# intel/pailliercryptolib

Hardware: AMD Instinct MI355X
Metric: 2048-bit modexps/sec (encrypt+decrypt) (higher is better)
Workload: dtype u64

## Files before the change

pailliercryptolib_amd/csrc/capi.cpp:

```cpp
#include "pgpu.h"

#include <hip/hip_runtime_api.h>

#include <algorithm>
#include <atomic>
#include <chrono>
#include <cstdio>
#include <cstdlib>
#include <cstring>
#include <deque>
#include <list>
#include <map>
#include <set>
#include <memory>
#include <mutex>
#include <string>
#include <vector>

#include "ipcl/bignum.h"
#include "kargs.hpp"
#include "launch.hpp"
#include "policy.hpp"
#include "runtime.hpp"

// ... 1490 lines not shown
               hipStream_t s, bool in_mont, const uint32_t* d_pair = nullptr, int in_pair_l2 = 0, int busy_lanes = 0) {
  const int nw = key->n_words;
  if (busy_lanes == 0 && key->hs_ps && hensel_enabled() && secret_policy() != PGPU_EXP_SLIDING &&
      (d_pair ? key->hs_ps->pair_l2 == in_pair_l2 : key->conv_form != nullptr)) {
    if (const size_t head = policy::ps_split_head(key->hs_ps->K, count)) {
      RC_TRY(decrypt_on(d, key, d_c, d_m, head, s, in_mont, d_pair, in_pair_l2, busy_lanes));
      return decrypt_on(d, key, d_c ? d_c + head * (size_t)2 * nw : nullptr, d_m + head * (size_t)nw, count - head, s, in_mont,
                        d_pair ? d_pair + head * (size_t)2 * in_pair_l2 : nullptr, in_pair_l2, busy_lanes);
    }
  }
  rt::StreamWork& w = d.work_for(s);
  std::lock_guard<std::mutex> lk(w.mu);
  RC_TRY(w.vbuf.ensure(2 * count * (size_t)nw * 8, s));
  const bool lat = use_latency_geo(key->geo_lat, key->geo_exp, 2 * count);
  const bool sliding = secret_policy() == PGPU_EXP_SLIDING && key->sched[0].dev.bytes;
  bool have_m = false;
  const pgpu_privkey::HenselSet* hset = pick_hensel(key, count);
  rt::DevMem conv_rows;
  if (!d_pair && !sliding && hset && key->conv_form) {
    const pgpu_privkey::HenselSet* cand = hset;
    const int cl2 = key->conv_form->H * key->conv_form->K;
    if (cand->pair_l2 == cl2 && (seq_form_pays(cand->H, cand->K, count, busy_lanes) || ps_form_pays(key, count, busy_lanes) ||
                                 wave_form_pays(key, count, busy_lanes))) {
      RC_TRY(conv_rows.alloc(d, s, count * (size_t)2 * cl2 * sizeof(uint32_t)));
      RC_TRY(words_to_pair_on(d, key->conv_form.get(), d_c, (size_t)2 * nw, 2 * nw, in_mont, (uint32_t*)conv_rows.p, count, s));
      d_pair = (const uint32_t*)conv_rows.p;
      in_pair_l2 = cl2;
    }
  }
  const bool wavef = d_pair && !sliding && hset && wave_form_pays(key, count, busy_lanes) && key->hs_ps->pair_l2 == in_pair_l2 &&
                     (policy::wave_policy() == 2 || 2 * count * (size_t)(1 + wave_neighbours(d, s)) <= kSimds);
  const bool psf = wavef || (d_pair && !sliding && hset && ps_form_pays(key, count, busy_lanes) &&
                             key->hs_ps->pair_l2 == in_pair_l2);
  if (psf) hset = key->hs_ps.get();
  const pgpu_privkey::HenselSet* bset = (psf && !wavef) ? ps_balanced_set(key, in_pair_l2) : nullptr;
  if (bset) hset = bset;
  if (d_pair && (!hset || hset->pair_l2 != in_pair_l2))
    return fail(PGPU_ERR_UNSUPPORTED, "decrypt: pair-row ciphertexts need the split-form kernel of this key size");
  if (hset) {
    const int L2 = hset->H * hset->K, nch = hset->nchunks, ipw = 64 / (2 * hset->H);
    const size_t side_words = hset->side_words();
    const uint32_t* blob = (const uint32_t*)hset->blob.d[(size_t)d.index];
    pgpu::HenselArgs h{};
    for (int sd = 0; sd < 2; ++sd) {
      const uint32_t* b = blob + sd * side_words;
      h.ctx[sd].nhat = b;
      h.ctx[sd].n = b + L2;
      h.ctx[sd].h = b + 2 * L2;
      h.ctx[sd].kr = b + 3 * L2;
      h.ctx[sd].one = b + 4 * L2;
      h.ctx[sd].conv = b + 6 * L2 + (in_mont ? (size_t)nch * 2 * L2 : 0);
      h.ctx[sd].n0inv = hset->n0inv[sd];
    }
    h.ct = d_c;
    h.ct_stride = (size_t)2 * nw;
    h.ct_words = 2 * nw;
    if (d_pair) {
      h.ct_pair = d_pair;
      h.ct_pair_stride = (size_t)2 * in_pair_l2;
      h.pair_l2 = in_pair_l2;
      h.pchunk_limbs = hset->pchunk_limbs;
      h.pchunks = hset->pchunks;
      for (int sd = 0; sd < 2; ++sd) {
        const uint32_t* pc = blob + sd * side_words + (size_t)L2 * (6 + 4 * (size_t)nch);
        h.ctx[sd].pconv = pc;
        h.ctx[sd].pcb = pc + (size_t)hset->pchunks * 2 * L2;
      }
    }
    h.chunk_words = hset->chunk_words;
    h.nchunks = nch;
    h.exp = (const uint64_t*)key->d_exps.d[(size_t)d.index];
    h.exp_stride = (size_t)key->pq_words;
    h.exp_words = key->pq_words;
    h.exp_bits = key->exp_bits;
    size_t entries;
    if (sliding) {
      for (int i = 0; i < 2; ++i) {
        h.sched[i] = (const uint16_t*)key->sched[i].dev.d[(size_t)d.index];
        h.sched_len[i] = key->sched[i].len;
      }
      h.window = key->sched[0].w;
      entries = (size_t)1 << (h.window - 1);
    } else {
      h.window = g_ct_gather.load() ? std::min(masked_decrypt_window(), pick_window(h.exp_bits)) : policy::pick_decrypt_window(h.exp_bits, 2 * count * (size_t)2 * L2 * sizeof(uint32_t));
      if (wavef) h.window = std::min(h.window, 5);
      entries = (size_t)1 << h.window;
    }
    h.ct_gather = g_ct_gather.load();
    h.out = (uint64_t*)w.vbuf.p;
    h.out_stride = (size_t)key->pq_words;
    h.out_words = key->pq_words;
    h.count = count;
    const size_t waves = 2 * ((count + ipw - 1) / ipw);
    const unsigned blocks = (unsigned)((waves + pgpu::kWavesPerWG - 1) / pgpu::kWavesPerWG);
    TimerScope t(d, s, PGPU_KERNEL_MODEXP);
    const size_t seq_ipw = 64 / (size_t)hset->H;
    const size_t seq_waves = 2 * ((count + seq_ipw - 1) / seq_ipw);
    const bool seq = !psf && d_pair && !sliding && seq_form_pays(hset->H, hset->K, count, busy_lanes);
    t.set_form(psf ? PGPU_FORM_LANE | PGPU_FORM_PS : seq ? PGPU_FORM_SEQ : PGPU_FORM_PAIRED);
    if (wavef) {
      t.set_form(PGPU_FORM_WAVE | PGPU_FORM_PS);
      RC_TRY(w.table.ensure(2 * count * (size_t)(2 * hset->pchunks) * pgpu::hensel_wave_pair_words(hset->K) * sizeof(uint32_t), s));
      h.table = (uint32_t*)w.table.p;
      static const bool wide_ok = [] { const char* e = getenv("PGPU_WAVE_WIDEQ"); return !e || atoi(e) != 0; }();
      const bool wide = wide_ok && hset->lb * hset->K - (key->exp_bits + hset->lb) >= 10;
      if (!pgpu::launch_hensel_wave(hset->K, hset->lb, wide, h, s))
        return fail(PGPU_ERR_UNSUPPORTED, "wavefront-wide decrypt kernel not compiled");
    } else if (psf) {
      const size_t lwaves = 2 * ((count + 63) / 64);
      const unsigned lblocks = (unsigned)((lwaves + pgpu::kWavesPerWG - 1) / pgpu::kWavesPerWG);
      RC_TRY(w.table.ensure((size_t)lblocks * pgpu::kWavesPerWG * pgpu::hensel_ps_table_words(hset->K, entries) * sizeof(uint32_t), s));
      h.table = (uint32_t*)w.table.p;
      const unsigned lds_pad = adaptive_cu_claim(lwaves, busy_lanes);
      if (lds_pad) t.set_form(PGPU_FORM_LANE | PGPU_FORM_PS | PGPU_FORM_CU_CLAIM);
      if (bset ? !pgpu::launch_hensel_psb(hset->K, hset->lb, h, lblocks, s, lds_pad)
               : !pgpu::launch_hensel_ps(hset->K, hset->lb, h, lblocks, s, lds_pad))
        return fail(PGPU_ERR_UNSUPPORTED, "one-lane product-scanning decrypt kernel not compiled");
    } else if (seq) {
      const unsigned sblocks = (unsigned)((seq_waves + pgpu::kWavesPerWG - 1) / pgpu::kWavesPerWG);
      RC_TRY(w.table.ensure((size_t)sblocks * pgpu::kWavesPerWG * seq_ipw * entries * 2 * L2 * sizeof(uint32_t), s));
      h.table = (uint32_t*)w.table.p;
      static const int env_pad = [] {
        const char* e = getenv("PGPU_SEQ_LDS_PAD");
        return e ? atoi(e) : -1;
      }();
      const int pol = policy::seq_policy();
      const unsigned lds_pad = env_pad >= 0 ? (unsigned)env_pad
                               : (seq_waves < kSimds && (pol == 3 || (pol == 4 && busy_lanes >= 1 && busy_lanes <= policy::adapt_claim_busy())) ? 84000u : 0u);
      if (lds_pad) t.set_form(PGPU_FORM_SEQ | PGPU_FORM_CU_CLAIM);
      static const bool w1 = [] { const char* e = getenv("PGPU_SEQ_W1"); return !e || atoi(e) != 0; }();
      if (!pgpu::launch_hensel_seq(hset->H, hset->K, h, sblocks, s, lds_pad, w1 && lds_pad >= 82000u))
        return fail(PGPU_ERR_UNSUPPORTED, "sequential-halves decrypt kernel not compiled");
    } else {
      RC_TRY(w.table.ensure((size_t)blocks * pgpu::kWavesPerWG * ipw * entries * 2 * L2 * sizeof(uint32_t), s));
      h.table = (uint32_t*)w.table.p;
      if (!pgpu::launch_hensel(hset->H, hset->K, waves > kSimds || g_packed_decrypt.load(), h, blocks, s))
        return fail(PGPU_ERR_UNSUPPORTED, "split-form kernel not compiled");
    }
    HIP_TRY(hipGetLastError());
    t.stop();
    have_m = true;
  }
  pgpu::ModexpArgs a{};
  const int vf = in_mont ? VF_BASE_MONT : VF_NONE;
  a.ctx[0] = (lat ? key->p2l : key->p2)->view(d.index, vf);
  a.ctx[1] = (lat ? key->q2l : key->q2)->view(d.index, vf);
  a.nctx = 2;
  a.base = d_c;
  a.base_stride = (size_t)2 * nw;
  a.base_words = 2 * nw;
  a.exp = (const uint64_t*)key->d_exps.d[(size_t)d.index];
  a.exp_stride = (size_t)key->pq_words;
  a.exp_per_ctx = 1;
  a.exp_words = key->pq_words;
  a.exp_bits = key->exp_bits;
  a.final_mul = pgpu::FM_CTX_CONST;
  a.out = (uint64_t*)w.vbuf.p;
  a.out_stride = (size_t)nw;
  a.count = 2 * count;
  SchedRef sr;
  if (sliding) {
    for (int i = 0; i < 2; ++i) {
      sr.p[i] = (const uint16_t*)key->sched[i].dev.d[(size_t)d.index];
      sr.len[i] = key->sched[i].len;
    }
    sr.w = key->sched[0].w;
  }
// ... 378 lines not shown
  *split = 0;
  *lanes = g.G;
  *limbs = g.K;
  return PGPU_OK;
}

int pgpu_decrypt_kernel_form(const pgpu_privkey* key, size_t count, int* split, int* lanes, int* limbs) {
  RC_TRY(pgpu_decrypt_kernel_form_ex(key, count, 0, split, lanes, limbs));
  if (*split == 4 && key->hs_ps) *limbs = key->hs_ps->K;
  return PGPU_OK;
}
int pgpu_decrypt_kernel_form_ex(const pgpu_privkey* key, size_t count, int busy_lanes, int* split, int* lanes, int* limbs) {
  if (!key || !split || !lanes || !limbs) return fail(PGPU_ERR_INVALID_PARAM, "pgpu_decrypt_kernel_form: bad argument");
  RC_TRY(check_gen(key->gen, "key"));
  if (const pgpu_privkey::HenselSet* f = pick_hensel(key, count)) {
    if (pair_rows_enabled() && secret_policy() != PGPU_EXP_SLIDING && wave_form_pays(key, count, busy_lanes) &&
        key->hs_ps->pair_l2 == f->pair_l2) {
      *split = 5;
      *lanes = 64;
      *limbs = key->hs_ps->K;
      return PGPU_OK;
    }
    if (pair_rows_enabled() && secret_policy() != PGPU_EXP_SLIDING && ps_form_pays(key, count, busy_lanes) &&
        key->hs_ps->pair_l2 == f->pair_l2) {
      *split = 4;
      *lanes = 1;
      const pgpu_privkey::HenselSet* bal = ps_balanced_set(key, f->pair_l2);
      *limbs = bal ? bal->K : key->hs_ps->K;
      return PGPU_OK;
    }
    if (pair_rows_enabled() && secret_policy() != PGPU_EXP_SLIDING && seq_form_pays(f->H, f->K, count, busy_lanes)) {
      *split = 2;
      *lanes = f->H;
    } else {
      *split = 1;
      *lanes = 2 * f->H;
    }
    *limbs = f->K;
    return PGPU_OK;
  }
  const bool lat = use_latency_geo(key->geo_lat, key->geo_exp, 2 * count);
  const GeoInfo g = lat ? key->geo_lat : launch_geo(key->geo_exp, 2 * count);
  *split = 0;
  *lanes = g.G;
  *limbs = g.K;
  return PGPU_OK;
}

int pgpu_set_fixed_base_window(int w) {
  if (w < 0 || w > kFbMaxW) return fail(PGPU_ERR_INVALID_PARAM, "fixed-base window must be 0..14");
  g_fb_window.store(w);
  g_fb_window_explicit.store(true);
  return PGPU_OK;
}

int pgpu_set_secret_exponent_policy(int policy) {
  if (policy != PGPU_EXP_FIXED_WINDOW && policy != PGPU_EXP_SLIDING)
    return fail(PGPU_ERR_INVALID_PARAM, "unknown exponent policy");
  g_secret_policy.store(policy);
  return PGPU_OK;
}
int pgpu_get_secret_exponent_policy(void) { return secret_policy(); }
int pgpu_set_table_gather_policy(int masked) {
  g_ct_gather.store(masked ? 1 : 0);
  return PGPU_OK;
}
int pgpu_get_table_gather_policy(void) { return g_ct_gather.load(); }

void pgpu_debug_set_wave_clocks(uint64_t* d_buf) { g_wave_clocks = d_buf; }
void pgpu_debug_set_row_source(int mode) { g_row_source.store(mode < 0 ? -1 : (mode ? 1 : 0)); }
void pgpu_debug_set_hensel(int mode) { g_hensel.store(mode < 0 ? 0 : (mode > 3 ? 3 : mode)); }
void pgpu_debug_set_packed_decrypt(int on) { g_packed_decrypt.store(on != 0); }
void pgpu_debug_set_seq_decrypt(int policy) { pgpu::policy::set_seq_policy(policy); }
int pgpu_debug_set_host_adapt(int on) {
  const int was = g_host_adapt.exchange(on != 0 ? 1 : 0);
  return was;
}
int pgpu_debug_get_seq_decrypt(void) { return pgpu::policy::seq_policy(); }
void pgpu_debug_set_ps_decrypt(int policy) { pgpu::policy::set_ps_policy(policy); }
void pgpu_debug_set_wave_decrypt(int policy) { pgpu::policy::set_wave_policy(policy); }
int pgpu_debug_get_wave_decrypt(void) { return pgpu::policy::wave_policy(); }
int pgpu_debug_get_ps_decrypt(void) { return pgpu::policy::ps_policy(); }
int pgpu_debug_set_ps_balanced(int on) { return g_ps_balanced.exchange(on != 0 ? 1 : 0); }
int pgpu_debug_set_rr_adapt(int min_busy) { return pgpu::policy::set_rr_adapt(min_busy); }

#include "capi_timing.inc"

int pgpu_dev_alloc(size_t bytes, void** out) {
  RC_TRY(rt::check_ready());
  return rt::current().alloc(bytes, nullptr, out);
}
void pgpu_dev_free(void* d_ptr) {
  if (!d_ptr) return;
  if (!rt::initialized()) {
    (void)hipFree(d_ptr);
    return;
  }
  rt::current().free(d_ptr, nullptr);
}
int pgpu_copy_h2d(void* d_dst, const void* h_src, size_t bytes) {
  RC_TRY(rt::check_ready());
  rt::TaskGroup tg;
  tg.run(rt::current(), [=](rt::Lane& lane) -> int {
    HIP_TRY(hipStreamSynchronize(nullptr));
    RC_TRY(lane.h2d(d_dst, h_src, bytes, lane.stream));
    HIP_TRY(hipStreamSynchronize(lane.stream));
    return PGPU_OK;
  });
  return tg.wait();
}
int pgpu_copy_d2h(void* h_dst, const void* d_src, size_t bytes) {
  RC_TRY(rt::check_ready());
  rt::TaskGroup tg;
  tg.run(rt::current(), [=](rt::Lane& lane) -> int {
    hipError_t e = hipStreamSynchronize(nullptr);
    if (e != hipSuccess) return fail(PGPU_ERR_HIP, std::string("kernel failed: ") + hipGetErrorString(e));
    return lane.d2h(h_dst, d_src, bytes, lane.stream);
  });
  return tg.wait();
}

int pgpu_host_alloc(size_t bytes, void** out) { return rt::host_alloc(bytes, out); }
void pgpu_host_free(void* p) { rt::host_free(p); }
int pgpu_host_wait(const void* p) { return rt::host_wait(p); }

int pgpu_modexp_dev(const uint64_t* d_base, size_t base_stride, const uint64_t* d_exp,
                    size_t exp_stride, int exp_words, int exp_bits, const uint64_t* h_mod,
                    int mod_words, uint64_t* d_out, size_t count, void* hip_stream) {
  RC_TRY(rt::check_ready());
  if (count == 0) return PGPU_OK;
  if (!d_base || !d_exp || !d_out) return fail(PGPU_ERR_INVALID_PARAM, "null batch pointer");
  if (exp_words <= 0 || exp_bits < 0 || exp_bits > 64 * exp_words)
    return fail(PGPU_ERR_INVALID_PARAM, "exp_bits/exp_words inconsistent");
  if (base_stride != 0 && base_stride < (size_t)mod_words)
    return fail(PGPU_ERR_INVALID_PARAM, "base stride smaller than the modulus width");
  if (exp_stride != 0 && exp_stride < (size_t)exp_words)
    return fail(PGPU_ERR_INVALID_PARAM, "exponent stride smaller than exp_words");
  rt::Device& d = rt::current();
  rt::DeviceGuard g(d.ordinal);
  return modexp_on(d, d_base, base_stride, d_exp, exp_stride, exp_words, exp_bits, h_mod, mod_words, d_out, count,
                   (hipStream_t)hip_stream, nullptr, false, false, nullptr);
}

int pgpu_modexp(const uint64_t* base, size_t base_stride, const uint64_t* exp, size_t exp_stride,
                int exp_words, int exp_bits, const uint64_t* mod, int mod_words, uint64_t* out,
                size_t count) {
  RC_TRY(rt::check_ready());
  if (count == 0) return PGPU_OK;
  if (!base || !exp || !out || mod_words <= 0 || exp_words <= 0)
    return fail(PGPU_ERR_INVALID_PARAM, "null batch pointer or zero width");
  if (exp_bits < 0 || exp_bits > 64 * exp_words)
    return fail(PGPU_ERR_INVALID_PARAM, "exp_bits/exp_words inconsistent");
  if (base_stride != 0 && base_stride < (size_t)mod_words)
    return fail(PGPU_ERR_INVALID_PARAM, "base stride smaller than the modulus width");
  if (exp_stride != 0 && exp_stride < (size_t)exp_words)
    return fail(PGPU_ERR_INVALID_PARAM, "exponent stride smaller than exp_words");
  std::shared_ptr<ModCtx> ctx;
  RC_TRY(get_modctx(mod, mod_words, true, &ctx));
  std::vector<uint16_t> sched;
  int sched_w = 0;
  if (exp_stride == 0 && count >= 16 && exp_bits > 8 && sliding_enabled()) {
    BigNumber e = BigNumber::fromLimbs64(exp, (size_t)exp_words);
    if (!e.isZero()) {
      sched_w = pick_sliding_window(e.BitSize());
      sched = sliding_schedule(e, sched_w);
    }
// ... 230 lines not shown
```

pailliercryptolib_amd/csrc/hensel_ps.hpp:

```cpp
#ifndef PAILLIERCRYPTOLIB_AMD_CSRC_HENSEL_PS_HPP_
#define PAILLIERCRYPTOLIB_AMD_CSRC_HENSEL_PS_HPP_

#include <utility>

#include "hensel.hpp"

#ifndef PGPU_PS_PIN
#define PGPU_PS_PIN 1
#endif
#ifndef PGPU_PS_SPLIT
#define PGPU_PS_SPLIT 0
#endif

namespace pgpu {

template <int LB>
struct PsLimb {
  static constexpr uint32_t mask = (1u << LB) - 1;
};

template <class F, int... Is>
__device__ __forceinline__ void ps_static_for_impl(F&& f, std::integer_sequence<int, Is...>) {
  (f(std::integral_constant<int, Is>{}), ...);
}
// ... 328 lines not shown
      b[j] = kb[j];
      ma[j] = HCTX(h)[j];
      mb[j] = 0;
    }
  }
  ps_pairmul<K, LB, false>(a, b, ma, mb, np, 0, n0, slot);
  uint32_t d[K];
  const uint32_t below_a = ps_sub<K, LB>(d, a, np);
  const uint32_t jflag = below_a ^ 1u;
  const uint32_t below = ps_sub<K, LB>(d, b, np);
  if (!below) {
#pragma unroll
    for (int j = 0; j < K; ++j) b[j] = d[j];
  }
  (void)ps_sub<K, LB>(d, np, b);
  {
    uint32_t jf[K];
#pragma unroll
    for (int j = 0; j < K; ++j) jf[j] = j == 0 ? jflag : 0u;
    ps_add<K, LB>(d, jf);
  }
  const uint32_t small = ps_sub<K, LB>(b, d, np);
  if (small) {
#pragma unroll
    for (int j = 0; j < K; ++j) b[j] = d[j];
  }
  if (live) {
    uint64_t* out = A.out + (2 * elem + side) * A.out_stride;
    const int ow = A.out_words;
    ps_static_for<W64>([&](auto wc) __attribute__((always_inline)) {
      constexpr int ww = decltype(wc)::value;
      if (ww < ow) out[ww] = ps_word<K, LB, ww>(b);
    });
    for (int ww = W64; ww < ow; ++ww) out[ww] = 0;
  }
#undef HCTX
}

template <int K>
constexpr size_t ps_table_words(size_t entries) { return entries * 2 * ((K + 3) / 4) * kWave * 4; }

template <int K, int LB, int MINW>
__global__ __launch_bounds__(kWGThreads, MINW) void hensel_decrypt_ps_kernel(HenselArgs A) {
  constexpr int K4 = (K + 3) / 4;
  raise_wave_priority();
  __shared__ uint4 park_[kWavesPerWG][K4][kWave];
  const int lane = threadIdx.x % kWave, wv = threadIdx.x / kWave;
  uint4* slot = &park_[wv][0][lane];
  const size_t wave_id = (size_t)blockIdx.x * kWavesPerWG + wv;
  const int side = __builtin_amdgcn_readfirstlane((int)(wave_id & 1));
  const size_t first_elem = (wave_id >> 1) * kWave;
  size_t elem = first_elem + lane;
  if (elem >= A.count) elem = A.count - 1;
#define HCTX(field) (side ? A.ctx[1].field : A.ctx[0].field)
  uint32_t n[K], a[K], b[K], ma[K], mb[K];
#pragma unroll
  for (int j = 0; j < K; ++j) n[j] = ps_uniform(HCTX(nhat)[j]);
  const uint32_t n1p = n[1] + 1;
  const int w = A.window, tsize = 1 << w;
  uint4* tw = reinterpret_cast<uint4*>(A.table + wave_id * ps_table_words<K>((size_t)tsize)) + lane;
  const uint64_t* ep = A.exp + (size_t)side * A.exp_stride;
  const int nwin = (A.exp_bits + w - 1) / w;
  auto digit = [&](int i) -> int {
    int bit = i * w;
    int word = bit >> 6, sh = bit & 63;
    uint64_t v = (word < A.exp_words) ? ep[word] >> sh : 0;
    if (sh + w > 64 && word + 1 < A.exp_words) v |= ep[word + 1] << (64 - sh);
    return (int)(v & (uint64_t)(tsize - 1));
  };
  const bool gather = A.ct_gather != 0;

  ps_entry_from_pair_row<K, LB>(A, side, elem, n, n1p, slot, a, b, ma, mb);
  ps_table_store<K>(tw, 1, a, b);
  {
    uint32_t oa[K], ob[K];
#pragma unroll
    for (int j = 0; j < K; ++j) {
      oa[j] = HCTX(one)[j];
      ob[j] = HCTX(one)[K + j];
    }
    ps_table_store<K>(tw, 0, oa, ob);
  }
#pragma unroll 1
  for (int e = 2; e < tsize; ++e) {
    ps_table_load<K>(ma, mb, tw, 1, tsize, false);
    ps_pairmul<K, LB, true>(a, b, ma, mb, n, n1p, 0, slot);
    ps_table_store<K>(tw, e, a, b);
  }
  int win = nwin - 2;
  if (nwin > 0) {
    ps_table_load<K>(a, b, tw, digit(nwin - 1), tsize, gather);
  } else {
#pragma unroll
    for (int j = 0; j < K; ++j) {
      a[j] = HCTX(one)[j];
      b[j] = HCTX(one)[K + j];
    }
  }
#pragma unroll 1
  for (; nwin > 0 && win >= 0; --win) {
    const int idx = digit(win);
#pragma unroll 1
    for (int i = 0; i < w; ++i) ps_pairsqr<K, LB>(a, b, n, n1p);
    ps_table_load<K>(ma, mb, tw, idx, tsize, gather);
    ps_pairmul<K, LB, true>(a, b, ma, mb, n, n1p, 0, slot);
  }
  ps_exit_words<K, LB>(A, side, elem, first_elem + lane < A.count, slot, a, b, ma, mb);
#undef HCTX
}

}

#endif
```

pailliercryptolib_amd/csrc/hensel_ps_bal.hpp:

```cpp
#ifndef PAILLIERCRYPTOLIB_AMD_CSRC_HENSEL_PS_BAL_HPP_
#define PAILLIERCRYPTOLIB_AMD_CSRC_HENSEL_PS_BAL_HPP_

#include "hensel_ps.hpp"

namespace pgpu {

template <int LB>
__device__ __forceinline__ int32_t psb_sext(uint32_t v) { return __builtin_amdgcn_sbfe((int)v, 0u, (unsigned)LB); }

__device__ __forceinline__ void psb_mac(int64_t& acc, int32_t x, int32_t y) { acc += (int64_t)x * y; }
__device__ __forceinline__ void psb_mac_pinned(int64_t& acc, int32_t x, int32_t y) {
  acc += (int64_t)x * y;
  asm volatile("" ::"v"(acc));
}

template <int K, int LB>
struct PsbFits {
  static constexpr bool value = 2 * (LB - 1) < 62 && LB + 6 < 62 &&
                                3 * (uint64_t)K * ((uint64_t)1 << (2 * (LB - 1))) + ((uint64_t)1 << (LB + 6)) < ((uint64_t)1 << 63);
};

template <int K, int LB, int NP, bool SYM, int QMODE>
__device__ __forceinline__ void psb_montmul(int32_t (&r)[K], const int32_t (&x1)[K], const int32_t (&y1)[K],
                                            const int32_t (&x2)[K], const int32_t (&y2)[K], const int32_t (&n)[K],
                                            uint32_t n0inv, int32_t (&qio)[K]) {
  static_assert(!(SYM && NP != 1), "a symmetric product is a single one");
  static_assert(PsbFits<K, LB>::value, "a column sums up to 3K products below 2^(2(LB-1)): must stay below 2^63");
  int32_t q[K];
  int64_t acc = 0;
  int32_t onev = 1;
  asm("" : "+v"(onev));
  ps_static_for<2 * K>([&](auto colc) __attribute__((always_inline)) {
    constexpr int col = decltype(colc)::value;
    {
      constexpr int ilo = col < K ? 0 : col - K + 1;
      constexpr int ihi = col < K ? col : K;
      if constexpr (ihi > ilo) {
        ps_static_for<ihi - ilo>([&](auto ic) __attribute__((always_inline)) {
          constexpr int i = ilo + decltype(ic)::value;
          if constexpr (PGPU_PS_PIN == 2 || (PGPU_PS_PIN == 1 && SYM)) psb_mac_pinned(acc, q[i], n[col - i]);
          else psb_mac(acc, q[i], n[col - i]);
        });
      }
    }
    if constexpr (SYM) {
      constexpr int ilo = col < K ? 0 : col - K + 1;
      constexpr int ihi = (col + 1) / 2;
      if constexpr (ihi > ilo) {
        int64_t cross = 0;
        ps_static_for<ihi - ilo>([&](auto ic) __attribute__((always_inline)) {
          constexpr int i = ilo + decltype(ic)::value;
          psb_mac(cross, x1[i], x1[col - i]);
        });
        acc = (int64_t)((uint64_t)acc + ((uint64_t)cross << 1));
      }
      if constexpr (col % 2 == 0) psb_mac(acc, x1[col / 2], x1[col / 2]);
    } else {
      constexpr int ilo = col < K ? 0 : col - K + 1;
      constexpr int ihi = col < K ? col + 1 : K;
      ps_static_for<ihi - ilo>([&](auto ic) __attribute__((always_inline)) {
        constexpr int i = ilo + decltype(ic)::value;
        if constexpr (PGPU_PS_PIN == 2) {
          psb_mac_pinned(acc, x1[i], y1[col - i]);
          if constexpr (NP == 2) psb_mac_pinned(acc, x2[i], y2[col - i]);
        } else {
          psb_mac(acc, x1[i], y1[col - i]);
          if constexpr (NP == 2) psb_mac(acc, x2[i], y2[col - i]);
        }
      });
    }
    if constexpr (col < K) {
      if constexpr (QMODE == 2) psb_mac(acc, qio[col], onev);
      q[col] = psb_sext<LB>((uint32_t)acc * n0inv);
      psb_mac(acc, q[col], n[0]);
      acc >>= LB;
      if constexpr (QMODE == 1) qio[col] = q[col];
    } else {
      r[col - K] = psb_sext<LB>((uint32_t)acc);
      if constexpr (col + 1 < 2 * K) acc = (acc + ((int64_t)1 << (LB - 1))) >> LB;
    }
  });
}

template <int K>
__device__ __forceinline__ uint32_t (&psb_bits(int32_t (&v)[K]))[K] { return reinterpret_cast<uint32_t(&)[K]>(v); }
template <int K>
__device__ __forceinline__ const uint32_t (&psb_bits(const int32_t (&v)[K]))[K] { return reinterpret_cast<const uint32_t(&)[K]>(v); }

template <int K, int LB>
__device__ __forceinline__ void psb_pairsqr(int32_t (&a)[K], int32_t (&b)[K], const int32_t (&n)[K], uint32_t n0inv) {
  int32_t qd[K], t[K];
  psb_montmul<K, LB, 1, true, 1>(t, a, a, a, a, n, n0inv, qd);
#pragma unroll
  for (int j = 0; j < K; ++j) b[j] *= 2;
  psb_montmul<K, LB, 1, false, 2>(b, a, b, a, b, n, n0inv, qd);
#pragma unroll
  for (int j = 0; j < K; ++j) a[j] = t[j];
}

template <int K, int LB>
__device__ __forceinline__ void psb_pairmul(int32_t (&a)[K], int32_t (&b)[K], const int32_t (&c)[K], const int32_t (&d)[K],
                                            const int32_t (&n)[K], uint32_t n0inv, uint4* slot) {
  int32_t qd[K];
  {
    int32_t t[K];
    ps_park_store<K>(slot, psb_bits<K>(b));
    __builtin_amdgcn_sched_barrier(0);
    psb_montmul<K, LB, 1, false, 1>(t, a, c, a, c, n, n0inv, qd);
    __builtin_amdgcn_sched_barrier(0);
    ps_park_swap<K>(slot, psb_bits<K>(b), psb_bits<K>(t));
    __builtin_amdgcn_sched_barrier(0);
  }
  psb_montmul<K, LB, 2, false, 2>(b, a, d, b, c, n, n0inv, qd);
  __builtin_amdgcn_sched_barrier(0);
  ps_park_load<K>(psb_bits<K>(a), slot);
}

template <int K, int LB>
__device__ __forceinline__ void psb_mul(int32_t (&r)[K], const int32_t (&x)[K], const int32_t (&y)[K], const int32_t (&n)[K],
                                        uint32_t n0inv) {
  int32_t none[K];
  psb_montmul<K, LB, 1, false, 0>(r, x, y, x, y, n, n0inv, none);
}

template <int K, int LB>
__device__ __forceinline__ void psb_add(int32_t (&a)[K], const int32_t (&k)[K]) {
  int32_t c = 0;
#pragma unroll
  for (int j = 0; j < K; ++j) {
    const int32_t u = a[j] + k[j] + c;
    a[j] = j + 1 < K ? psb_sext<LB>((uint32_t)u) : u;
    c = (u + (1 << (LB - 1))) >> LB;
  }
}

template <int K, int LB, int NI>
__device__ __forceinline__ void psb_relimb(int32_t (&out)[K], const uint32_t (&in)[NI]) {
  static_assert(NI <= K, "the chunk must fit");
  uint32_t c = 0;
#pragma unroll
  for (int j = 0; j < K; ++j) {
    const uint32_t u = (j < NI ? in[j] : 0u) + c;
    out[j] = j + 1 < K ? psb_sext<LB>(u) : (int32_t)u;
    c = (u + (1u << (LB - 1))) >> LB;
  }
}

template <int K, int LB>
__device__ __forceinline__ int32_t psb_canon(uint32_t (&out)[K], const int32_t (&v)[K]) {
  int32_t c = 0;
#pragma unroll
  for (int j = 0; j < K; ++j) {
    const int32_t u = v[j] + c;
    out[j] = (uint32_t)u & PsLimb<LB>::mask;
    c = u >> LB;
  }
  return c;
}

template <int K, int LB>
__device__ __forceinline__ void psb_entry_from_pair_row(const HenselArgs& A, int side, size_t elem, const int32_t (&n)[K],
                                                        uint32_t n0inv, uint4* slot, int32_t (&a)[K], int32_t (&b)[K],
                                                        int32_t (&ma)[K], int32_t (&mb)[K]) {
  static_assert(LB == kLimbBits, "the row limbs are re-balanced, not re-cut");
  constexpr int NI = (K * LB - 2) / LB + 1;
#define HCTX(field) (side ? A.ctx[1].field : A.ctx[0].field)
  const uint32_t* row = A.ct_pair + elem * A.ct_pair_stride;
  int32_t acc_a[K], acc_b[K];
#pragma unroll
  for (int j = 0; j < K; ++j) acc_a[j] = acc_b[j] = 0;
#pragma unroll 1
  for (int i = 0; i < A.pchunks; ++i) {
    const int first = i * A.pchunk_limbs;
    uint32_t za[NI], zb[NI];
    int32_t cb[K], tb[K];
#pragma unroll
    for (int j = 0; j < NI; ++j) {
      const bool in = j < A.pchunk_limbs && first + j < A.pair_l2;
// ... 24 lines not shown
#undef HCTX
}

template <int K, int LB>
__device__ __forceinline__ void psb_exit_words(const HenselArgs& A, int side, size_t elem, bool live, uint4* slot,
                                               const int32_t (&n)[K], uint32_t n0inv, int32_t (&a)[K], int32_t (&b)[K],
                                               int32_t (&ma)[K], int32_t (&mb)[K]) {
  constexpr int W64 = (K * LB + 63) / 64;
#define HCTX(field) (side ? A.ctx[1].field : A.ctx[0].field)
#pragma unroll
  for (int j = 0; j < K; ++j) {
    ma[j] = (int32_t)HCTX(h)[j];
    mb[j] = 0;
  }
  psb_pairmul<K, LB>(a, b, ma, mb, n, n0inv, slot);
  uint32_t u0[K], u1[K];
  const int32_t neg_a = psb_canon<K, LB>(u0, a);
#pragma unroll
  for (int j = 0; j < K; ++j) ma[j] = a[j] - n[j];
  const int32_t below_p = psb_canon<K, LB>(u0, ma);
  const int32_t jflag = (below_p + 1) + neg_a;
#pragma unroll
  for (int j = 0; j < K; ++j) ma[j] = (j == 0 ? jflag : 0) - b[j];
  const int32_t neg_d = psb_canon<K, LB>(u0, ma);
#pragma unroll
  for (int j = 0; j < K; ++j) ma[j] += n[j];
  (void)psb_canon<K, LB>(u1, ma);
#pragma unroll
  for (int j = 0; j < K; ++j) u0[j] = neg_d ? u1[j] : u0[j];
  if (live) {
    uint64_t* out = A.out + (2 * elem + side) * A.out_stride;
    const int ow = A.out_words;
    ps_static_for<W64>([&](auto wc) __attribute__((always_inline)) {
      constexpr int ww = decltype(wc)::value;
      if (ww < ow) out[ww] = ps_word<K, LB, ww>(u0);
    });
    for (int ww = W64; ww < ow; ++ww) out[ww] = 0;
  }
#undef HCTX
}

template <int K, int LB, int MINW>
__global__ __launch_bounds__(kWGThreads, MINW) void hensel_decrypt_psb_kernel(HenselArgs A) {
  constexpr int K4 = (K + 3) / 4;
  raise_wave_priority();
  __shared__ uint4 park_[kWavesPerWG][K4][kWave];
  const int lane = threadIdx.x % kWave, wv = threadIdx.x / kWave;
  uint4* slot = &park_[wv][0][lane];
  const size_t wave_id = (size_t)blockIdx.x * kWavesPerWG + wv;
  const int side = __builtin_amdgcn_readfirstlane((int)(wave_id & 1));
  const size_t first_elem = (wave_id >> 1) * kWave;
  size_t elem = first_elem + lane;
  if (elem >= A.count) elem = A.count - 1;
#define HCTX(field) (side ? A.ctx[1].field : A.ctx[0].field)
  int32_t n[K], a[K], b[K], ma[K], mb[K];
#pragma unroll
  for (int j = 0; j < K; ++j) n[j] = (int32_t)ps_uniform(HCTX(nhat)[j]);
  const uint32_t n0inv = ps_uniform(HCTX(n0inv));
  const int w = A.window, tsize = 1 << w;
  uint4* tw = reinterpret_cast<uint4*>(A.table + wave_id * ps_table_words<K>((size_t)tsize)) + lane;
  const uint64_t* ep = A.exp + (size_t)side * A.exp_stride;
  const int nwin = (A.exp_bits + w - 1) / w;
  auto digit = [&](int i) -> int {
    int bit = i * w;
    int word = bit >> 6, sh = bit & 63;
    uint64_t v = (word < A.exp_words) ? ep[word] >> sh : 0;
    if (sh + w > 64 && word + 1 < A.exp_words) v |= ep[word + 1] << (64 - sh);
    return (int)(v & (uint64_t)(tsize - 1));
  };
  const bool gather = A.ct_gather != 0;

  psb_entry_from_pair_row<K, LB>(A, side, elem, n, n0inv, slot, a, b, ma, mb);
  ps_table_store<K>(tw, 1, psb_bits<K>(a), psb_bits<K>(b));
  {
    uint32_t oa[K], ob[K];
#pragma unroll
    for (int j = 0; j < K; ++j) {
      oa[j] = HCTX(one)[j];
      ob[j] = HCTX(one)[K + j];
    }
    ps_table_store<K>(tw, 0, oa, ob);
  }
#pragma unroll 1
  for (int e = 2; e < tsize; ++e) {
    ps_table_load<K>(psb_bits<K>(ma), psb_bits<K>(mb), tw, 1, tsize, false);
    psb_pairmul<K, LB>(a, b, ma, mb, n, n0inv, slot);
    ps_table_store<K>(tw, e, psb_bits<K>(a), psb_bits<K>(b));
  }
  int win = nwin - 2;
  if (nwin > 0) {
    ps_table_load<K>(psb_bits<K>(a), psb_bits<K>(b), tw, digit(nwin - 1), tsize, gather);
  } else {
#pragma unroll
    for (int j = 0; j < K; ++j) {
      a[j] = (int32_t)HCTX(one)[j];
      b[j] = (int32_t)HCTX(one)[K + j];
    }
  }
#pragma unroll 1
  for (; nwin > 0 && win >= 0; --win) {
    const int idx = digit(win);
#pragma unroll 1
    for (int i = 0; i < w; ++i) psb_pairsqr<K, LB>(a, b, n, n0inv);
    ps_table_load<K>(psb_bits<K>(ma), psb_bits<K>(mb), tw, idx, tsize, gather);
    psb_pairmul<K, LB>(a, b, ma, mb, n, n0inv, slot);
  }
  psb_exit_words<K, LB>(A, side, elem, first_elem + lane < A.count, slot, n, n0inv, a, b, ma, mb);
#undef HCTX
}

}

#endif
```

pailliercryptolib_amd/csrc/policy.cpp:

```cpp
#include "policy.hpp"

#include <algorithm>
#include <atomic>
#include <cstdlib>
#include <utility>

#include "launch.hpp"

namespace pgpu {
namespace policy {

namespace {
int env_int(const char* name, int dflt, int lo, int hi) {
  const char* e = std::getenv(name);
  return e ? std::max(lo, std::min(hi, std::atoi(e))) : dflt;
}
std::atomic<int> g_seq_policy{env_int("PGPU_SEQ_DECRYPT", 4, 0, 4)};
std::atomic<int> g_ps_policy{env_int("PGPU_PS_DECRYPT", 1, 0, 2)};
constexpr int kAdaptEncSeq = 3;
constexpr int kAdaptClaimBusy = 3;
std::atomic<int> g_wave_policy{env_int("PGPU_WAVE_FORMS", 1, 0, 2)};
std::atomic<int> g_rr_adapt{env_int("PGPU_RR_ADAPT", 3, 0, 100)};
}

int seq_policy() { return g_seq_policy.load(); }
void set_seq_policy(int p) { g_seq_policy.store(p < 0 ? 0 : (p > 4 ? 4 : p)); }
int ps_policy() { return g_ps_policy.load(); }
void set_ps_policy(int p) { g_ps_policy.store(p < 0 ? 0 : (p > 2 ? 2 : p)); }
int adapt_claim_busy() { return kAdaptClaimBusy; }
int wave_policy() { return g_wave_policy.load(); }
void set_wave_policy(int p) { g_wave_policy.store(p < 0 ? 0 : (p > 2 ? 2 : p)); }
int rr_adapt() { return g_rr_adapt.load(); }
int set_rr_adapt(int min_busy) { return g_rr_adapt.exchange(min_busy < 0 ? 0 : min_busy); }

int seq_policy_by_size() {
  const int p = g_seq_policy.load();
  return (p == 3 || p == 4) ? 1 : p;
}
bool seq_adaptive(size_t waves, int busy) {
  return g_seq_policy.load() == 4 && busy >= 1 && waves * (size_t)(1 + busy) >= kSimds;
}
unsigned adaptive_cu_claim(size_t waves, int busy_lanes) {
  return (g_seq_policy.load() == 4 && waves < kSimds && busy_lanes >= 1 && busy_lanes <= kAdaptClaimBusy) ? 84000u : 0u;
}

bool fb_encrypt_seq_pays(int H, int K, size_t count, int busy) {
  if (!pgpu::hensel_fb_encrypt_seq_has(H, K)) return false;
  const size_t ipw = 64 / (size_t)H;
  const size_t waves = (count + ipw - 1) / ipw;
  const int pol = seq_policy_by_size();
  if (H == 4 && busy != 2 && busy <= kAdaptEncSeq && seq_adaptive(waves, busy)) return true;
  if (H == 2 && pol != 2) return false;
  return pol == 2 || (pol == 1 && waves >= (H >= 8 ? 2 : 1) * kSimds);
}
bool modexp_seq_form_pays(int H, int K, size_t count) {
  if (!pgpu::hensel_modexp_seq_has(H, K)) return false;
  const size_t ipw = 64 / (size_t)H;
  const size_t waves = (count + ipw - 1) / ipw;
  const int pol = seq_policy_by_size();
  if (H == 2 && pol != 2) return false;
  return pol == 2 || (pol == 1 && waves >= (H >= 8 ? 2 : 1) * kSimds);
}
bool seq_form_pays(int H, int K, size_t count, int busy) {
  if (!pgpu::hensel_seq_has(H, K)) return false;
  const size_t ipw = 64 / (size_t)H;
  const size_t waves = 2 * ((count + ipw - 1) / ipw);
  const int pol = g_seq_policy.load();
  return pol == 2 || (pol == 3 && 2 * waves >= kSimds) || ((pol == 1 || pol == 4) && waves >= kSimds) || seq_adaptive(waves, busy);
}
size_t ps_min_count(int K) {
  return K == 56 ? 24576 + 1 : (K == 38 || K == 19) ? 16384 + 1 : kPsRound;
}
static size_t ps_split_tail(int K) { return K == 56 ? 24576 : 16384; }
bool wave_form_pays(size_t count, int busy) {
  const int pol = g_wave_policy.load();
  if (pol == 2) return true;
  return pol == 1 && g_ps_policy.load() == 1 && busy == 0 && 2 * count <= kSimds;
}
bool modexp_wave_form_pays(size_t count) {
  const int pol = g_wave_policy.load();
  if (pol == 2) return true;
  return pol == 1 && g_ps_policy.load() == 1 && count <= kSimds;
}
bool ps_form_pays(size_t count, int busy, int K) {
  const size_t waves = 2 * ((count + 63) / 64);
  const int pol = g_ps_policy.load();
  return pol == 2 || (pol == 1 && (count >= ps_min_count(K) || seq_adaptive(waves, busy)));
}
size_t ps_split_head(int K, size_t count) {
  if (g_ps_policy.load() != 1 || count <= kPsRound) return 0;
  const size_t tail = count % kPsRound;
  return (tail != 0 && tail <= ps_split_tail(K)) ? count - tail : 0;
}
bool pair_mul_seq_pays(int H, int K, size_t count) {
  if (!pgpu::pair_mul_seq_has(H, K)) return false;
  const size_t ipw = 64 / (size_t)H;
  const size_t waves = (count + ipw - 1) / ipw;
  const int pol = seq_policy_by_size();
  return pol == 2 || (pol == 1 && waves >= (H >= 8 ? 2 : 1) * kSimds);
}

int pick_window(int exp_bits) {
  static const int forced = env_int("PGPU_FIXED_WINDOW", 0, 1, 6);
  if (forced) return forced;
  int best = 1;
  long best_cost = 1L << 60;
  for (int w = 1; w <= 5; ++w) {
    long cost = ((1L << w) - 2) + (exp_bits + w - 1) / w;
    if (cost < best_cost) { best_cost = cost; best = w; }
  }
  return best;
}
constexpr size_t kDecryptTableCap = (size_t)4 << 30;
int pick_decrypt_window(int exp_bits, size_t entry_bytes) {
  const int w5 = pick_window(exp_bits);
  static const int forced = env_int("PGPU_FIXED_WINDOW", 0, 1, 6);
  if (forced || exp_bits < 1280) return w5;
  if (entry_bytes > (kDecryptTableCap >> 6)) return w5;
  const long c5 = ((1L << w5) - 2) + (exp_bits + w5 - 1) / w5, c6 = ((1L << 6) - 2) + (exp_bits + 5) / 6;
  return c6 < c5 ? 6 : w5;
}
int masked_decrypt_window() { return 3; }

static long env_now(const char* name) {
  const char* e = std::getenv(name);
  return e && *e ? std::atol(e) : 0;
}
bool pair_form_for_bits(int n_bits, int* G, int* K) {
  static const int forms[4][2] = {{2, 19}, {4, 18}, {8, 14}, {8, 18}};
  if (n_bits < 1) return false;
  for (const auto& f : forms) {
    if (pgpu::kLimbBits * f[0] * f[1] >= n_bits + pgpu::kLimbBits + 8 && pgpu::pair_ops_has(f[0], f[1])) {
      if (G) *G = f[0];
      if (K) *K = f[1];
      return true;
    }
  }
  return false;
}
bool pair_wide_form(int G, int K, int* wide_G, int* wide_K) {
  if (K % 2 != 0 || !pgpu::pair_ops_alt_has(2 * G, K / 2)) return false;
  if (wide_G) *wide_G = 2 * G;
  if (wide_K) *wide_K = K / 2;
  return true;
}
void pub_forms_for_bits(int n_bits, std::vector<std::pair<int, int>>* forms) {
  forms->clear();
  if (n_bits < 1) return;
  const int need = n_bits + pgpu::kLimbBits + 8, nsq_bits = 2 * n_bits;
  int PG = 0, PK = 0, WG = 0, WK = 0;
  const bool has_pair = pair_form_for_bits(n_bits, &PG, &PK);
  const bool has_wide = has_pair && pair_wide_form(PG, PK, &WG, &WK);
  for (int H : {8, 4, 2})
    for (int K = 1; K <= 19; ++K)
      if ((pgpu::hensel_modexp_has(H, K) || pgpu::hensel_fb_has(H, K)) && pgpu::kLimbBits * H * K >= need &&
          2 * pgpu::kLimbBits * H * K >= nsq_bits + 8) {
        if (!(has_pair && H == PG && K == PK) && !(has_wide && H == WG && K == WK)) forms->push_back({H, K});
        break;
      }
  if (has_wide) forms->push_back({WG, WK});
  if (has_pair) forms->push_back({PG, PK});
}
bool matvec_geometry(int key_bits, int* G, int* K) {
  int g = 0, k = 0;
  if (!pair_form_for_bits(key_bits, &g, &k) || !pgpu::matvec_has(g, k)) return false;
  if (G) *G = g;
  if (K) *K = k;
  return true;
}
size_t matvec_slices(int G, size_t rows, size_t cols) {
  if (rows == 0 || cols == 0) return 1;
  const long forced = env_now("PGPU_MATVEC_SLICES");
  if (forced > 0) return std::min((size_t)forced, cols);
  const size_t ipw = 64 / (size_t)G;
  const size_t row_waves = (rows + ipw - 1) / ipw;
  const size_t fill = (kSimds + row_waves - 1) / row_waves;
  const size_t cap = std::max<size_t>(1, cols / kMatvecMinSliceCols);
  return std::max<size_t>(1, std::min(std::min(fill, cap), cols));
}
double matvec_products(size_t rows, size_t cols, int e_bits, int w, size_t slices) {
  const double nwin = (double)((e_bits + w - 1) / w);
  return (double)cols * (double)(((size_t)1 << w) - 2) + (double)rows * (double)slices * (double)e_bits +
         (double)rows * (double)cols * nwin + (double)rows * (double)(slices - 1);
}
int matvec_window(size_t rows, size_t cols, int e_bits, size_t slices, size_t row_bytes) {
  const long forced = env_now("PGPU_MATVEC_WINDOW");
  if (forced > 0) return (int)std::min(forced, 6L);
  int best = 1;
  double best_cost = matvec_products(rows, cols, e_bits, 1, slices);
  for (int w = 2; w <= 6; ++w) {
    if ((double)cols * (double)((size_t)1 << w) * (double)row_bytes > (double)kMatvecTableCap) break;
    const double cost = matvec_products(rows, cols, e_bits, w, slices);
    if (cost < best_cost) { best_cost = cost; best = w; }
  }
  return best;
}


bool segsum_sort(const uint32_t* ids, size_t groups, size_t cols, size_t n_segments, std::vector<uint32_t>* perm,
                 std::vector<size_t>* offsets) {
// ... 160 lines not shown
```

pailliercryptolib_amd/csrc/policy.hpp:

```cpp
#ifndef PAILLIERCRYPTOLIB_AMD_CSRC_POLICY_HPP_
#define PAILLIERCRYPTOLIB_AMD_CSRC_POLICY_HPP_

#include <stddef.h>
#include <stdint.h>

#include <utility>
#include <vector>

#include "kargs.hpp"

namespace pgpu {
namespace policy {

constexpr size_t kSimds = 256 * 4;
constexpr size_t kRrAdaptMinCount = 4096;

int seq_policy();
void set_seq_policy(int p);
int ps_policy();
void set_ps_policy(int p);
int adapt_claim_busy();
int wave_policy();
void set_wave_policy(int p);
int rr_adapt();
int set_rr_adapt(int min_busy);

int seq_policy_by_size();
bool seq_adaptive(size_t waves, int busy);
unsigned adaptive_cu_claim(size_t waves, int busy_lanes);
bool seq_form_pays(int H, int K, size_t count, int busy = 0);
constexpr size_t kPsRound = 32768;
size_t ps_min_count(int K);
bool ps_form_pays(size_t count, int busy, int K = 38);
size_t ps_split_head(int K, size_t count);
bool wave_form_pays(size_t count, int busy);
bool modexp_wave_form_pays(size_t count);
bool fb_encrypt_seq_pays(int H, int K, size_t count, int busy = 0);
bool modexp_seq_form_pays(int H, int K, size_t count);
bool pair_mul_seq_pays(int H, int K, size_t count);
int pick_window(int exp_bits);
int pick_decrypt_window(int exp_bits, size_t entry_bytes = 0);
int masked_decrypt_window();


bool pair_form_for_bits(int n_bits, int* G, int* K);
bool pair_wide_form(int G, int K, int* wide_G, int* wide_K);
void pub_forms_for_bits(int n_bits, std::vector<std::pair<int, int>>* forms);


bool matvec_geometry(int key_bits, int* G, int* K);
constexpr size_t kMatvecMinSliceCols = 4;
size_t matvec_slices(int G, size_t rows, size_t cols);
constexpr size_t kMatvecTableCap = (size_t)256 << 20;
int matvec_window(size_t rows, size_t cols, int e_bits, size_t slices, size_t row_bytes);
double matvec_products(size_t rows, size_t cols, int e_bits, int w, size_t slices);


constexpr uint32_t kSegsumNone = 0xFFFFFFFFu;
bool segsum_sort(const uint32_t* ids, size_t groups, size_t cols, size_t n_segments, std::vector<uint32_t>* perm,
                 std::vector<size_t>* offsets);
constexpr size_t kSegsumWavesPerSimd = 8;
constexpr size_t kSegsumMinChunk = 8;
constexpr size_t kSegsumMaxChunk = 256;
constexpr size_t kSegsumForcedMax = 65536;
int segsum_chunk(int G, size_t elements);
bool segsum_wide_pays(int wide_G, size_t chains);
int segsum_levels(int chunk, size_t longest);
struct SegsumLevel {
  std::vector<SegsumChunk> chunks;
  size_t partial_rows = 0;
};
struct SegsumPlan {
  int chunk = 0;
  size_t longest = 0;
  std::vector<SegsumLevel> levels;
};
void segsum_plan(const std::vector<size_t>& offsets, int chunk, SegsumPlan* plan);


constexpr size_t kSegscanWavesPerSimd = 8;
constexpr size_t kSegscanMinChunk = 8;
constexpr size_t kSegscanForcedMax = 65536;
int segscan_chunk(int G, size_t rows, size_t seg_len);
int segscan_levels(int chunk, size_t seg_len);
size_t segscan_products(int chunk, size_t rows, size_t seg_len);
bool segscan_fits(int chunk, size_t rows, size_t seg_len);
struct SegscanLevel {
  size_t rows = 0, seg_len = 0;
  bool reverse = false;
  std::vector<SegsumChunk> up;
  size_t totals = 0;
  std::vector<SegscanChunk> scan;
};
struct SegscanPlan {
  int chunk = 0;
  size_t products = 0;
  std::vector<SegscanLevel> levels;
};
void segscan_plan(size_t rows, size_t seg_len, int chunk, bool reverse, SegscanPlan* plan);


bool pack_wide_pays(int wide_G, size_t rows);
bool pack_geometry(int key_bits, size_t rows, int* G, int* K);

}
}

#endif
```

Baseline: 6.280 million.

## Build window tables with squarings and pre-double squaring operand in PS decrypt

The per-lane (PS) decrypt table build now produces even entries by squaring entry k, not by multiplying by the base each time, so half the builds use the cheaper squaring. In the balanced-limb path, the pair squaring doubles the operand once up front and reuses it for both the symmetric cross products and the second product, removing a separate doubling pass and the shift-add of the cross sum. The decrypt window picker gains a one-lane cost model weighted by separate squaring and multiplication instruction counts. This may choose a different window for the lane form, and it also makes the fixed-window override settable at runtime.

```diff
diff --git a/pailliercryptolib_amd/csrc/capi.cpp b/pailliercryptolib_amd/csrc/capi.cpp
--- a/pailliercryptolib_amd/csrc/capi.cpp
+++ b/pailliercryptolib_amd/csrc/capi.cpp
@@ -1596,7 +1596,7 @@
       h.window = key->sched[0].w;
       entries = (size_t)1 << (h.window - 1);
     } else {
-      h.window = g_ct_gather.load() ? std::min(masked_decrypt_window(), pick_window(h.exp_bits)) : policy::pick_decrypt_window(h.exp_bits, 2 * count * (size_t)2 * L2 * sizeof(uint32_t));
+      h.window = g_ct_gather.load() ? std::min(masked_decrypt_window(), pick_window(h.exp_bits)) : policy::pick_decrypt_window(h.exp_bits, 2 * count * (size_t)2 * L2 * sizeof(uint32_t), psf && !wavef);
       if (wavef) h.window = std::min(h.window, 5);
       entries = (size_t)1 << h.window;
     }
@@ -2141,6 +2141,10 @@
 int pgpu_debug_get_wave_decrypt(void) { return pgpu::policy::wave_policy(); }
 int pgpu_debug_get_ps_decrypt(void) { return pgpu::policy::ps_policy(); }
 int pgpu_debug_set_ps_balanced(int on) { return g_ps_balanced.exchange(on != 0 ? 1 : 0); }
+int pgpu_debug_set_fixed_window(int w) { return pgpu::policy::set_fixed_window(w); }
+int pgpu_debug_decrypt_window(int exp_bits, size_t entry_bytes, int one_lane) {
+  return pgpu::policy::pick_decrypt_window(exp_bits, entry_bytes, one_lane != 0);
+}
 int pgpu_debug_set_rr_adapt(int min_busy) { return pgpu::policy::set_rr_adapt(min_busy); }
 
 #include "capi_timing.inc"
diff --git a/pailliercryptolib_amd/csrc/hensel_ps.hpp b/pailliercryptolib_amd/csrc/hensel_ps.hpp
--- a/pailliercryptolib_amd/csrc/hensel_ps.hpp
+++ b/pailliercryptolib_amd/csrc/hensel_ps.hpp
@@ -434,10 +434,14 @@
     ps_table_store<K>(tw, 0, oa, ob);
   }
 #pragma unroll 1
-  for (int e = 2; e < tsize; ++e) {
+  for (int k = 1; 2 * k < tsize; ++k) {
+    ps_table_load<K>(a, b, tw, k, tsize, false);
+    ps_pairsqr<K, LB>(a, b, n, n1p);
+    ps_table_store<K>(tw, 2 * k, a, b);
+    __builtin_amdgcn_sched_barrier(0);
     ps_table_load<K>(ma, mb, tw, 1, tsize, false);
     ps_pairmul<K, LB, true>(a, b, ma, mb, n, n1p, 0, slot);
-    ps_table_store<K>(tw, e, a, b);
+    ps_table_store<K>(tw, 2 * k + 1, a, b);
   }
   int win = nwin - 2;
   if (nwin > 0) {
diff --git a/pailliercryptolib_amd/csrc/hensel_ps_bal.hpp b/pailliercryptolib_amd/csrc/hensel_ps_bal.hpp
--- a/pailliercryptolib_amd/csrc/hensel_ps_bal.hpp
+++ b/pailliercryptolib_amd/csrc/hensel_ps_bal.hpp
@@ -2,6 +2,10 @@
 #define PAILLIERCRYPTOLIB_AMD_CSRC_HENSEL_PS_BAL_HPP_
 
 #include "hensel_ps.hpp"
+
+#ifndef PGPU_PSB_DOUBLED
+#define PGPU_PSB_DOUBLED 1
+#endif
 
 namespace pgpu {
 
@@ -20,11 +24,12 @@
                                 3 * (uint64_t)K * ((uint64_t)1 << (2 * (LB - 1))) + ((uint64_t)1 << (LB + 6)) < ((uint64_t)1 << 63);
 };
 
-template <int K, int LB, int NP, bool SYM, int QMODE>
+template <int K, int LB, int NP, bool SYM, int QMODE, bool DBL = false>
 __device__ __forceinline__ void psb_montmul(int32_t (&r)[K], const int32_t (&x1)[K], const int32_t (&y1)[K],
                                             const int32_t (&x2)[K], const int32_t (&y2)[K], const int32_t (&n)[K],
                                             uint32_t n0inv, int32_t (&qio)[K]) {
   static_assert(!(SYM && NP != 1), "a symmetric product is a single one");
+  static_assert(SYM || !DBL, "the doubled operand belongs to the symmetric product");
   static_assert(PsbFits<K, LB>::value, "a column sums up to 3K products below 2^(2(LB-1)): must stay below 2^63");
   int32_t q[K];
   int64_t acc = 0;
@@ -46,15 +51,25 @@
     if constexpr (SYM) {
       constexpr int ilo = col < K ? 0 : col - K + 1;
       constexpr int ihi = (col + 1) / 2;
-      if constexpr (ihi > ilo) {
-        int64_t cross = 0;
-        ps_static_for<ihi - ilo>([&](auto ic) __attribute__((always_inline)) {
-          constexpr int i = ilo + decltype(ic)::value;
-          psb_mac(cross, x1[i], x1[col - i]);
-        });
-        acc = (int64_t)((uint64_t)acc + ((uint64_t)cross << 1));
+      if constexpr (DBL) {
+        if constexpr (ihi > ilo) {
+          ps_static_for<ihi - ilo>([&](auto ic) __attribute__((always_inline)) {
+            constexpr int i = ilo + decltype(ic)::value;
+            psb_mac(acc, x1[i], y1[col - i]);
+          });
+        }
+        if constexpr (col % 2 == 0) psb_mac(acc, y1[col / 2], y1[col / 2]);
+      } else {
+        if constexpr (ihi > ilo) {
+          int64_t cross = 0;
+          ps_static_for<ihi - ilo>([&](auto ic) __attribute__((always_inline)) {
+            constexpr int i = ilo + decltype(ic)::value;
+            psb_mac(cross, x1[i], x1[col - i]);
+          });
+          acc = (int64_t)((uint64_t)acc + ((uint64_t)cross << 1));
+        }
+        if constexpr (col % 2 == 0) psb_mac(acc, x1[col / 2], x1[col / 2]);
       }
-      if constexpr (col % 2 == 0) psb_mac(acc, x1[col / 2], x1[col / 2]);
     } else {
       constexpr int ilo = col < K ? 0 : col - K + 1;
       constexpr int ihi = col < K ? col + 1 : K;
@@ -87,13 +102,21 @@
 template <int K>
 __device__ __forceinline__ const uint32_t (&psb_bits(const int32_t (&v)[K]))[K] { return reinterpret_cast<const uint32_t(&)[K]>(v); }
 
-template <int K, int LB>
+template <int K, int LB, bool DBL = (PGPU_PSB_DOUBLED != 0)>
 __device__ __forceinline__ void psb_pairsqr(int32_t (&a)[K], int32_t (&b)[K], const int32_t (&n)[K], uint32_t n0inv) {
   int32_t qd[K], t[K];
-  psb_montmul<K, LB, 1, true, 1>(t, a, a, a, a, n, n0inv, qd);
-#pragma unroll
-  for (int j = 0; j < K; ++j) b[j] *= 2;
-  psb_montmul<K, LB, 1, false, 2>(b, a, b, a, b, n, n0inv, qd);
+  if constexpr (DBL) {
+    int32_t a2[K];
+#pragma unroll
+    for (int j = 0; j < K; ++j) a2[j] = a[j] * 2;
+    psb_montmul<K, LB, 1, true, 1, true>(t, a2, a, a2, a, n, n0inv, qd);
+    psb_montmul<K, LB, 1, false, 2>(b, a2, b, a2, b, n, n0inv, qd);
+  } else {
+    psb_montmul<K, LB, 1, true, 1>(t, a, a, a, a, n, n0inv, qd);
+#pragma unroll
+    for (int j = 0; j < K; ++j) b[j] *= 2;
+    psb_montmul<K, LB, 1, false, 2>(b, a, b, a, b, n, n0inv, qd);
+  }
 #pragma unroll
   for (int j = 0; j < K; ++j) a[j] = t[j];
 }
@@ -284,10 +307,14 @@
     ps_table_store<K>(tw, 0, oa, ob);
   }
 #pragma unroll 1
-  for (int e = 2; e < tsize; ++e) {
+  for (int k = 1; 2 * k < tsize; ++k) {
+    ps_table_load<K>(psb_bits<K>(a), psb_bits<K>(b), tw, k, tsize, false);
+    psb_pairsqr<K, LB>(a, b, n, n0inv);
+    ps_table_store<K>(tw, 2 * k, psb_bits<K>(a), psb_bits<K>(b));
+    __builtin_amdgcn_sched_barrier(0);
     ps_table_load<K>(psb_bits<K>(ma), psb_bits<K>(mb), tw, 1, tsize, false);
     psb_pairmul<K, LB>(a, b, ma, mb, n, n0inv, slot);
-    ps_table_store<K>(tw, e, psb_bits<K>(a), psb_bits<K>(b));
+    ps_table_store<K>(tw, 2 * k + 1, psb_bits<K>(a), psb_bits<K>(b));
   }
   int win = nwin - 2;
   if (nwin > 0) {
diff --git a/pailliercryptolib_amd/csrc/policy.cpp b/pailliercryptolib_amd/csrc/policy.cpp
--- a/pailliercryptolib_amd/csrc/policy.cpp
+++ b/pailliercryptolib_amd/csrc/policy.cpp
@@ -100,8 +100,11 @@
   return pol == 2 || (pol == 1 && waves >= (H >= 8 ? 2 : 1) * kSimds);
 }
 
+static std::atomic<int> g_fixed_window{env_int("PGPU_FIXED_WINDOW", 0, 1, 6)};
+int set_fixed_window(int w) { return g_fixed_window.exchange(w <= 0 ? 0 : std::min(w, 6)); }
+
 int pick_window(int exp_bits) {
-  static const int forced = env_int("PGPU_FIXED_WINDOW", 0, 1, 6);
+  const int forced = g_fixed_window.load();
   if (forced) return forced;
   int best = 1;
   long best_cost = 1L << 60;
@@ -112,10 +115,22 @@
   return best;
 }
 constexpr size_t kDecryptTableCap = (size_t)4 << 30;
-int pick_decrypt_window(int exp_bits, size_t entry_bytes) {
+constexpr long kPsSqrInstr = 5260, kPsMulInstr = 7278;
+int pick_decrypt_window(int exp_bits, size_t entry_bytes, bool one_lane) {
   const int w5 = pick_window(exp_bits);
-  static const int forced = env_int("PGPU_FIXED_WINDOW", 0, 1, 6);
-  if (forced || exp_bits < 1280) return w5;
+  if (g_fixed_window.load()) return w5;
+  if (one_lane) {
+    int best = 1;
+    long best_cost = 1L << 60;
+    for (int w = 1; w <= 6; ++w) {
+      if (w == 6 && entry_bytes > (kDecryptTableCap >> 6)) break;
+      const long nwin = (exp_bits + w - 1) / w, build = (1L << (w - 1)) - 1;
+      const long cost = ((nwin - 1) * w + build) * kPsSqrInstr + ((nwin - 1) + build) * kPsMulInstr;
+      if (cost < best_cost) { best_cost = cost; best = w; }
+    }
+    return best;
+  }
+  if (exp_bits < 1280) return w5;
   if (entry_bytes > (kDecryptTableCap >> 6)) return w5;
   const long c5 = ((1L << w5) - 2) + (exp_bits + w5 - 1) / w5, c6 = ((1L << 6) - 2) + (exp_bits + 5) / 6;
   return c6 < c5 ? 6 : w5;
diff --git a/pailliercryptolib_amd/csrc/policy.hpp b/pailliercryptolib_amd/csrc/policy.hpp
--- a/pailliercryptolib_amd/csrc/policy.hpp
+++ b/pailliercryptolib_amd/csrc/policy.hpp
@@ -39,7 +39,8 @@
 bool modexp_seq_form_pays(int H, int K, size_t count);
 bool pair_mul_seq_pays(int H, int K, size_t count);
 int pick_window(int exp_bits);
-int pick_decrypt_window(int exp_bits, size_t entry_bytes = 0);
+int pick_decrypt_window(int exp_bits, size_t entry_bytes = 0, bool one_lane = false);
+int set_fixed_window(int w);
 int masked_decrypt_window();
 
 
```

Result: faster. 6.350 million (median of 6 runs) (+1.1%).
